# theteamatx/x-edr-trajectory-planning

Hardware: AMD Instinct MI355X
Metric: time-optimal path timings/s (7-DOF, 2000 s-samples), 1/2/4/8 MI355X + %HBM roofline (higher is better)
Workload: dtype f64

## Files before the change

x-edr-trajectory-planning_amd/csrc/tpamd_device.h:

```cpp
#pragma once

#include <hip/hip_runtime.h>
#include <float.h>
#include <stdint.h>

namespace tpamd {

constexpr double kTiny = 2.220446049250313e-16 * 1e5;
constexpr double kMaxSd2 = 1e6;

enum : uint8_t { kBndNone = 0, kBndSource = 1, kBndSink = 2, kBndTrajectory = 4 };
enum : uint8_t { kBndEqualsZ00 = 8, kBndTypeMask = 7 };

enum : uint32_t {
  kErrInfeasible = 1u,
  kErrSRange = 2u,
  kErrSdStartNeg = 4u,
  kErrLowerGeUpper = 8u,
  kErrTooFew = 16u,
  kErrSkip = 32u
};

__device__ __forceinline__ bool is_tiny(double v) { return fabs(v) < kTiny; }
__device__ __forceinline__ double qnan() { return __longlong_as_double(0x7ff8000000000000LL); }

__device__ __forceinline__ int status_from_bits(uint32_t bits) {
  if (bits & kErrInfeasible) return 2;
  if (bits & kErrSRange) return 3;
  if (bits & kErrSdStartNeg) return 4;
  if (bits & kErrLowerGeUpper) return 5;
  if (bits & kErrTooFew) return 6;
  return 0;
}


struct LdsRows {
  const double *A, *B, *LO, *HI;
  int stride;
  int lim_stride;
  __device__ __forceinline__ double a(int c) const { return A[c * stride]; }
  __device__ __forceinline__ double b(int c) const { return B[c * stride]; }
  __device__ __forceinline__ double lo(int c) const { return LO[c * lim_stride]; }
  __device__ __forceinline__ double hi(int c) const { return HI[c * lim_stride]; }
};

struct LdsRowsJoint {
  const double *Q1, *Q2;
  const double *lim_lo, *lim_hi;
  int stride, D;
  int E = 0;
  const double *X = nullptr;
  __device__ __forceinline__ double a(int c) const { return c < D ? Q1[c * stride] : 0.0; }
  __device__ __forceinline__ double b(int c) const {
    if (c < D) return Q2[c * stride];
    if (c >= 2 * D) return X[(c - 2 * D) * stride];
    const double v = Q1[(c - D) * stride];
    return v * v;
  }
  __device__ __forceinline__ double lo(int c) const { return lim_lo[c]; }
  __device__ __forceinline__ double hi(int c) const { return lim_hi[c]; }
};

struct JointRowsAt {
  const double *q12;
  const double *lim_lo, *lim_hi;
  int D;
  int E = 0;
  __device__ __forceinline__ double a(int c) const { return c < D ? q12[2 * c] : 0.0; }
  __device__ __forceinline__ double b(int c) const {
    if (c < D) return q12[2 * c + 1];
    if (c >= 2 * D) return q12[c];
    const double v = q12[2 * (c - D)];
    return v * v;
  }
  __device__ __forceinline__ double lo(int c) const { return lim_lo[c]; }
  __device__ __forceinline__ double hi(int c) const { return lim_hi[c]; }
};

struct GlobalRowsAt {
  const double *A, *B, *LO, *HI;
  __device__ __forceinline__ double a(int c) const { return A[c]; }
  __device__ __forceinline__ double b(int c) const { return B[c]; }
  __device__ __forceinline__ double lo(int c) const { return LO[c]; }
  __device__ __forceinline__ double hi(int c) const { return HI[c]; }
};

template <class R>
__device__ __forceinline__ bool rows_valid(const R &r, int C, double sdd, double sd2) {
  for (int i = 0; i < C; i++) {
    const double v = r.a(i) * sdd + r.b(i) * sd2;
// ... 79 lines not shown
    double bs[D], hi[D];
#pragma unroll
    for (int j = 0; j < D; j++) { bs[j] = b[j] * sd2; hi[j] = lim_hi[j]; }
#pragma unroll
    for (int i = 0; i < D; i++) {
      const double A = a[i];
      if (!is_tiny(A)) {
#pragma unroll
        for (int w = 0; w < 2; w++) {
          const double lim = w ? hi[i] : -hi[i];
          const double sddi = (lim - bs[i]) / A;
          if ((fabs(sddi) <= DBL_MAX) && ((sddi > smax) || (sddi < smin))) {
            bool bad = false;
#pragma unroll
            for (int j = 0; j < D; j++) {
              const double v = a[j] * sddi + bs[j];
              bad = bad | (fabs(v) - kTiny > hi[j]);
            }
            if (!bad) {
              if (sddi > smax) smax = sddi;
              if (sddi < smin) smin = sddi;
            }
          }
        }
      }
    }
  }
  if (smax == -DBL_MAX) smax = 0;
  if (smin == DBL_MAX) smin = 0;
  *sdd_max = smax;
  *sdd_min = smin;
}

template <int D>
__device__ __forceinline__ void find_sdd_both_joint_screened(const double (&a)[D], const double (&b)[D],
                                                             const double *Q1, const double *Q2, int stride,
                                                             const double *lim_hi, double sd2,
                                                             double *sdd_max, double *sdd_min) {
  double smax = -DBL_MAX, smin = DBL_MAX;
  bool vel_bad = false;
#pragma unroll
  for (int j = 0; j < D; j++) {
    const double v = (a[j] * a[j]) * sd2;
    vel_bad = vel_bad | (v + kTiny < 0.0) | (v - kTiny > lim_hi[D + j]);
  }
  const bool vel_ok = !vel_bad;
  if (vel_ok) {
    double bs[D], hi[D], c_lo[D], c_hi[D];
    double Lmax = -DBL_MAX, Umin = DBL_MAX;
#pragma unroll
    for (int j = 0; j < D; j++) {
      bs[j] = b[j] * sd2;
      hi[j] = lim_hi[j];
      const double r = __builtin_amdgcn_rcp(a[j]);
      c_lo[j] = (-hi[j] - bs[j]) * r;
      c_hi[j] = (hi[j] - bs[j]) * r;
      const bool counts = !is_tiny(a[j]);
      const double pad = kTiny * fabs(r);
      const double l = fmin(c_lo[j], c_hi[j]) - pad, u = fmax(c_lo[j], c_hi[j]) + pad;
      Lmax = (counts & (l > Lmax)) ? l : Lmax;
      Umin = (counts & (u < Umin)) ? u : Umin;
    }
    unsigned survivors = 0;
#pragma unroll
    for (int i = 0; i < D; i++) {
      const bool counts = !is_tiny(a[i]);
#pragma unroll
      for (int w = 0; w < 2; w++) {
        const double c = w ? c_hi[i] : c_lo[i];
        const double mg = 1e-6 * (fabs(Lmax) + fabs(Umin) + fabs(c)) + 1e-290;
        const bool out = (c < Lmax - mg) | (c > Umin + mg);
        survivors |= (counts & !out) ? (1u << (2 * i + w)) : 0u;
      }
    }
    while (__any(survivors != 0u)) {
      const bool live = survivors != 0u;
      const int slot = live ? (__ffs((int)survivors) - 1) : 0;
      survivors &= survivors - 1u;
      const int i = slot >> 1;
      const double A = Q1[i * stride];
      const double lim = (slot & 1) ? lim_hi[i] : -lim_hi[i];
      const double sddi = (lim - Q2[i * stride] * sd2) / A;
      if (live && (fabs(sddi) <= DBL_MAX) && ((sddi > smax) || (sddi < smin))) {
        bool bad = false;
#pragma unroll
        for (int j = 0; j < D; j++) {
          const double v = a[j] * sddi + bs[j];
          bad = bad | (fabs(v) - kTiny > hi[j]);
        }
        if (!bad) {
          if (sddi > smax) smax = sddi;
          if (sddi < smin) smin = sddi;
        }
      }
    }
  }
  if (smax == -DBL_MAX) smax = 0;
  if (smin == DBL_MAX) smin = 0;
  *sdd_max = smax;
  *sdd_min = smin;
}

template <int WORDS>
struct SlotSet {
  uint64_t w[WORDS];
  __device__ __forceinline__ void clear() {
#pragma unroll
    for (int i = 0; i < WORDS; i++) w[i] = 0;
  }
  __device__ __forceinline__ void fill(int n) {
#pragma unroll
    for (int i = 0; i < WORDS; i++) {
      const int lo = i * 64;
      w[i] = (n >= lo + 64) ? ~0ull : (n > lo ? ((1ull << (n - lo)) - 1ull) : 0ull);
    }
// ... 54 lines not shown
__device__ __forceinline__ bool lp_cannot_pass(double num, double den, double lo_lim,
                                               double hi_lim) {
  const double tmp_apx = num * __builtin_amdgcn_rcp(den);
  return (tmp_apx > hi_lim + fabs(hi_lim) * 1e-6) || (tmp_apx < lo_lim - fabs(lo_lim) * 1e-6);
}

template <class R>
__device__ __forceinline__ bool lp_pair_optimal(const R &r, int s1, int s2) {
  const int first = s1 >> 1, second = s2 >> 1;
  const bool first_upper = !(s1 & 1), second_upper = !(s2 & 1);
  const double a1 = r.a(first), a2 = r.a(second);
  const double denom = a2 * r.b(first) - a1 * r.b(second);
  const double t1 = denom * a1;
  const double t2 = denom * (-a2);
  const bool c1 = second_upper ? (t1 <= 0) : (t1 >= 0);
  const bool c2 = first_upper ? (t2 <= 0) : (t2 >= 0);
  return !(fabs(denom) < kTiny) & c1 & c2;
}

template <int WORDS, class R, int SD = 0, int SC = 0>
__device__ void lp_find_max_sd2(const R &r, int C, double *sd2max, double *sddmax,
                                double *sd2zero, int b_only_from = -1,
                                const double *ra = nullptr, const double *rb = nullptr) {
  typedef SlotSet<WORDS> Set;
  Set cset, act;
  cset.fill(2 * C);
  if (b_only_from >= 0) cset.drop_lower_from(b_only_from, C);
  act.clear();

  auto vel_b = [&](int c) -> double {
    if (SD > 0 && c < 2 * SD) { const double v = ra[c - SD]; return v * v; }
    return r.b(c);
  };
  double sd2 = DBL_MAX, sdd = 0.0;
  double hi_w = (sd2 + kTiny) + fabs(sd2 + kTiny) * 1e-6;
  auto step2_row = [&](int c, double Bc) {
    const bool pos = Bc > kTiny, neg = Bc < -kTiny;
    const double lim = pos ? r.hi(c) : r.lo(c);
    const double ap = lim * __builtin_amdgcn_rcp(Bc);
    if ((pos | neg) & !((ap > hi_w) | (ap < 0.0))) {
      const double invB = 1.0 / Bc;
      const double tmp = lim * invB;
      if (tmp < (sd2 + kTiny) && tmp > 0) {
        if (tmp < sd2 - kTiny) act.clear();
        act.set(2 * c + (pos ? 0 : 1));
        sd2 = tmp;
        hi_w = (sd2 + kTiny) + fabs(sd2 + kTiny) * 1e-6;
      }
    }
  };
  if (SD > 0) {
#pragma unroll
    for (int c = 0; c < SC; c++) step2_row(c, (c < SD) ? rb[c < SD ? c : 0] : vel_b(c));
  } else {
    for (int c = 0; c < C; c++) step2_row(c, r.b(c));
  }
  if (sd2 > kMaxSd2 || !act.any()) {
    *sd2zero = kMaxSd2;
    *sd2max = kMaxSd2;
    *sddmax = 0.0;
    return;
  }
  *sd2zero = sd2;

  int search = act.next(0);
  if (act.count() >= 2) {
    double best_slope = fabs(r.a(search >> 1) * (1.0 / r.b(search >> 1)));
    for (int s1 = act.next(0); s1 >= 0; s1 = act.next(s1 + 1)) {
      const double slope = fabs(r.a(s1 >> 1) * (1.0 / r.b(s1 >> 1)));
      if (slope < best_slope) {
        best_slope = slope;
        search = s1;
      }
      for (int s2 = act.next(s1 + 1); s2 >= 0; s2 = act.next(s2 + 1)) {
        if (lp_pair_optimal(r, s1, s2)) {
          *sd2max = sd2;
          *sddmax = 0.0;
          return;
        }
      }
    }
  }
  cset.remove(act);

  for (int loop = 0; loop < C; loop++) {
    if (search < 0) break;
    const int sc = search >> 1;
    const double As = r.a(sc);
    if (fabs(As) < kTiny) {
      *sd2max = sd2;
      *sddmax = sdd;
      return;
    }
    const double invA = 1.0 / As;
    const double b = -r.b(sc) * invA;
    const double a = (search & 1) ? r.lo(sc) * invA : r.hi(sc) * invA;

    act.clear();
    double next_sd2 = DBL_MAX, next_sdd = 0.0;
    const double lo_w = sd2 - fabs(sd2) * 1e-6;
    double up_w = (next_sd2 + kTiny) + fabs(next_sd2 + kTiny) * 1e-6;
    auto visit = [&](int s, bool member, double Ac, double Brow, double lim) {
      const double Bc = Ac * b + Brow;
      const double num = lim - Ac * a;
      const double tmp_apx = num * __builtin_amdgcn_rcp(Bc);
      if (!(member & !(fabs(Bc) < kTiny) & !((tmp_apx > up_w) | (tmp_apx < lo_w)))) return;
      const double invB = 1.0 / Bc;
      const double tmp = num * invB;
      if (tmp < (next_sd2 + kTiny) && tmp > sd2) {
        if (tmp < next_sd2 - kTiny) act.clear();
        act.set(s);
        next_sd2 = tmp;
        next_sdd = a + b * next_sd2;
        up_w = (next_sd2 + kTiny) + fabs(next_sd2 + kTiny) * 1e-6;
      }
    };
    if (SD > 0) {
#pragma unroll
      for (int c = 0; c < SC; c++) {
        const double Ac = (c < SD) ? ra[c < SD ? c : 0] : r.a(c);
        const double Brow = (c < SD) ? rb[c < SD ? c : 0] : vel_b(c);
        visit(2 * c, cset.has(2 * c), Ac, Brow, r.hi(c));
        if (!(b_only_from >= 0 && c >= b_only_from)) visit(2 * c + 1, cset.has(2 * c + 1), Ac, Brow, r.lo(c));
      }
    } else {
      for (int s = cset.next(0); s >= 0; s = cset.next(s + 1)) {
        const int c = s >> 1;
        visit(s, true, r.a(c), r.b(c), (s & 1) ? r.lo(c) : r.hi(c));
      }
    }
    if (!act.any()) {
      *sd2max = *sd2zero;
      *sddmax = 0.0;
      return;
    }
    const int old_search = search;
    search = -1;
    double best_slope = DBL_MAX;
    for (int s1 = act.next(0); s1 >= 0; s1 = act.next(s1 + 1)) {
      const int c1 = s1 >> 1;
      const double Ac = r.a(c1);
      const double slope = fabs(Ac * (1.0 / (Ac * b + r.b(c1))));
      if (slope < best_slope) {
        best_slope = slope;
        search = s1;
      }
      bool opt = false;
      for (int s2 = act.next(s1 + 1); s2 >= 0 && !opt; s2 = act.next(s2 + 1))
        opt = lp_pair_optimal(r, s1, s2);
      if (!opt) opt = lp_pair_optimal(r, s1, old_search);
      if (opt) {
        *sd2max = next_sd2;
        *sddmax = next_sdd;
        if (next_sd2 > kMaxSd2) {
          *sd2max = kMaxSd2;
          *sddmax = 0.0;
// ... 122 lines not shown
```

x-edr-trajectory-planning_amd/csrc/tpamd_capi.hip:

```cpp
#include "../../include/tpamd.h"

#include <hip/hip_runtime.h>

#include <algorithm>
#include <cmath>
#include <cstdio>
#include <cstdlib>
#include <cstring>
#include <mutex>
#include <new>
#include <vector>

#include "tpamd_kernels.h"
#include "tpamd_launch.h"
#include "tpamd_planner_set.h"
#include "tpamd_readout.h"
#include "tpamd_rescale.h"
#include "tpamd_buffer.h"
#include "tpamd_stop.h"
#include "tpamd_switch.h"
#include "tpamd_fit.h"
#include "tpamd_pose_fit.h"
#include "tpamd_sweep_joint.h"

// ... 326 lines not shown
};

struct DeviceScope {
  int prev = -1;
  hipError_t err;
  explicit DeviceScope(int device) {
    if (hipGetDevice(&prev) != hipSuccess) prev = -1;
    err = (prev == device) ? hipSuccess : hipSetDevice(device);
    if (prev == device) prev = -1;
  }
  ~DeviceScope() {
    if (prev >= 0) (void)hipSetDevice(prev);
  }
};
#define TPAMD_ON_DEVICE(e)          \
  DeviceScope device_scope_((e)->device); \
  HIPCHK(device_scope_.err)

constexpr int kMaxDevices = 64;
std::mutex g_config_mutex;
bool g_device_configured[kMaxDevices] = {};

template <typename K>
hipError_t allow_big_lds(K kernel, int bytes = 160 * 1024) {
  return hipFuncSetAttribute(reinterpret_cast<const void *>(kernel),
                             hipFuncAttributeMaxDynamicSharedMemorySize, bytes);
}

int configure_kernels_for_device(int device) {
  if (device < 0 || device >= kMaxDevices) return TPAMD_E_INVALID_ARGUMENT;
  std::lock_guard<std::mutex> lock(g_config_mutex);
  if (g_device_configured[device]) return 0;
#define TPAMD_BIG_LDS(...) HIPCHK(allow_big_lds(__VA_ARGS__))
  TPAMD_BIG_LDS(k_sample_lp_joint<1, 0>);
  TPAMD_BIG_LDS(k_sample_lp_joint<1, 3>);
  TPAMD_BIG_LDS(k_sample_lp_joint<1, 4>);
  TPAMD_BIG_LDS(k_sample_lp_joint<1, 5>);
  TPAMD_BIG_LDS(k_sample_lp_joint<1, 6>);
  TPAMD_BIG_LDS(k_sample_lp_joint<1, 7>);
  TPAMD_BIG_LDS(k_sample_lp_joint<1, 8>);
  TPAMD_BIG_LDS(k_sample_lp_joint<1, 14>);
  TPAMD_BIG_LDS(k_sample_lp_joint_wide<1, 14>);
  TPAMD_BIG_LDS(k_lp_rows<1>);
  TPAMD_BIG_LDS(k_lp_rows<2>);
  TPAMD_BIG_LDS(k_sweep<JointSource>);
  TPAMD_BIG_LDS(k_sweep<GenericSource>);
#define TPAMD_CONFIGURE_SWEEP(D, E) HIPCHK((configure_sweep_joint<D, E>()));
  TPAMD_SWEEP_INSTANCES(TPAMD_CONFIGURE_SWEEP)
#undef TPAMD_CONFIGURE_SWEEP
  TPAMD_BIG_LDS(k_cartesian_lp<1, 6>);
  TPAMD_BIG_LDS(k_cartesian_lp<1, 7>);
  TPAMD_BIG_LDS(k_resample_skip, 128 * 1024);
#undef TPAMD_BIG_LDS
  g_device_configured[device] = true;
  return 0;
}

bool has_joint_sweep(int D) { return (D >= 3 && D <= 8) || D == 14; }

template <class Source>
bool launch_sweep(hipStream_t st, int B, int N, int max_loops, const Source &src,
                  const Workspace &ws, const tpamd_path_outputs *out, bool ) {
  const size_t lds = (2 * (size_t)N + 64) * sizeof(double);
  hipLaunchKernelGGL((k_sweep<Source>), dim3(B), dim3(64), lds, st, N, max_loops, src, ws,
                     out->time, out->s, out->sd, out->sdd, out->last_extremal_index,
                     out->max_time_increment, out->status);
  return false;
}

template <>
bool launch_sweep<JointSource>(hipStream_t st, int B, int N, int max_loops, const JointSource &src,
                               const Workspace &ws, const tpamd_path_outputs *out,
                               bool force_generic) {
#define TPAMD_LAUNCH_JOINT(DD)                                              \
  do {                                                                      \
// ... 213 lines not shown
  return rc;
}

size_t tpamd_engine_workspace_bytes(const tpamd_engine *e) { return e ? e->ws_buf.bytes : 0; }

}

namespace {
int joint_args(const tpamd_joint_batch *bt, const tpamd_joint_inputs *in, const tpamd_path_outputs *out) {
  const int D = bt->num_dofs, N = bt->num_samples, P = bt->num_points;
  if (D < 1 || D > 16 || N < 3 || N > 8192 || P < 3) return TPAMD_E_UNSUPPORTED;
  if (!in->knots || !in->control_points || !in->max_velocity || !in->max_acceleration ||
      !in->path_start || !in->delta || !in->sd_start || !in->time_start || !out->time ||
      !out->s || !out->sd || !out->sdd || !out->status)
    return TPAMD_E_INVALID_ARGUMENT;
  return 0;
}

int solve_joint(tpamd_engine *e, const tpamd_joint_batch *bt, const tpamd_joint_inputs *in,
                const tpamd_path_outputs *out, void *hip_stream, const PlanParams *plan,
                bool allow_pipelining = true) {
  if (!e || !bt || !in || !out) return TPAMD_E_INVALID_ARGUMENT;
  const int B = bt->num_paths, D = bt->num_dofs, N = bt->num_samples, P = bt->num_points;
  if (B <= 0) return B == 0 ? 0 : TPAMD_E_INVALID_ARGUMENT;
  if (int rc = joint_args(bt, in, out)) return rc;
  TPAMD_ON_DEVICE(e);
  hipStream_t st = (hipStream_t)hip_stream;
  const int C = 2 * D;
  bool piped = e->pipelining != 0 && plan == nullptr && allow_pipelining;
  if (piped && stream_is_capturing(st)) piped = false;
  int tpb = piped ? 128 : (D <= 7 ? 256 : (D < 14 ? 128 : 64));
  if (!piped && in->num_samples_per_path && tpb > e->k1_tpb_ragged) tpb = e->k1_tpb_ragged;
  if (e->k1_tpb == 64 || e->k1_tpb == 128 || e->k1_tpb == 256) tpb = e->k1_tpb;
  const size_t lds = ((size_t)(P + 3) + (size_t)P * D + 2 * C + 2 * (size_t)D * tpb) * 8;
  if (lds > 160 * 1024) return TPAMD_E_UNSUPPORTED;
  if (piped) select_slot(e, 1 - e->slot);
  const int slot = e->slot;
  SlotGuard slot_guard(e, st, true, !piped);
  int rc = ensure_workspace(e, B, N, C);
  if (rc) return rc;
  e->last_B = B; e->last_N = N; e->last_time = out->time;
  e->ws.ns = in->num_samples_per_path;
  e->ws.amax = in->max_acceleration;
  e->ws.np = plan ? plan->np : nullptr;
  e->ws.p_stride = (plan && plan->np) ? plan->K - 3 : P;
  int32_t *order = const_cast<int32_t *>(e->ws.order);
  const bool ordered = in->num_samples_per_path != nullptr && B > 1 && e->order_ragged && plan == nullptr;
  if (!ordered) e->ws.order = nullptr;
  const Workspace &ws = e->ws;
  const int max_loops = bt->max_solver_loops > 0 ? bt->max_solver_loops : 0;
  hipStream_t fs = st;
  if (piped) {
    fs = e->aux;
    HIPCHK(hipStreamWaitEvent(fs, e->ev_sweep[slot], 0));
  }
  const bool do_front = e->phase != 2, do_back = e->phase != 1;
  if (do_front && piped && e->front_delay_us > 0)
    hipLaunchKernelGGL(k_delay, dim3(1), dim3(64), 0, fs, e->front_delay_us * 100);
  if (do_front) {
    Timer t(e, fs, KI_SETUP);
    hipLaunchKernelGGL(k_setup_joint, dim3((B + 127) / 128), dim3(128), 0, fs, B, N, D,
                       bt->constraint_safety, in->max_velocity, in->max_acceleration,
                       in->path_start, in->delta, in->sd_start, in->sdd_start, in->time_start,
                       ws);
    if (plan)
      hipLaunchKernelGGL(k_plan_mark_skipped, dim3((B + 127) / 128), dim3(128), 0, fs, *plan, ws);
    if (ordered)
      hipLaunchKernelGGL(k_order_paths, dim3(1), dim3(1024), 0, fs, B, N, in->num_samples_per_path, order);
  }
  if (do_front && e->front_wait) HIPCHK(hipStreamWaitEvent(fs, e->front_wait, 0));
  if (do_front) {
    Timer t(e, fs, KI_SAMPLE_LP);
    const dim3 grid((N + tpb - 1) / tpb, B);
#define TPAMD_K1(DD)                                                                         \
  hipLaunchKernelGGL((k_sample_lp_joint<1, DD>), grid, dim3(tpb), lds, fs, N, D, P, in->knots, \
                     in->control_points, out->q, ws)
    if (D == 7 && !e->force_generic) TPAMD_K1(7);
    else if (D == 6 && !e->force_generic) TPAMD_K1(6);
    else if (D == 14 && !e->force_generic)
      hipLaunchKernelGGL((k_sample_lp_joint_wide<1, 14>), grid, dim3(tpb), lds, fs, N, D, P, in->knots,
                         in->control_points, out->q, ws);
    else if (D == 3 && !e->force_generic) TPAMD_K1(3);
    else if (D == 4 && !e->force_generic) TPAMD_K1(4);
    else if (D == 5 && !e->force_generic) TPAMD_K1(5);
    else if (D == 8 && !e->force_generic) TPAMD_K1(8);
    else TPAMD_K1(0);
#undef TPAMD_K1
    if (plan) hipLaunchKernelGGL(k_plan_project, dim3((B + 127) / 128), dim3(128), 0, fs, *plan, ws);
  }
  if (do_front && e->front_record) HIPCHK(hipEventRecord(e->front_record, fs));
  if (!do_back) {
    HIPCHK(hipGetLastError());
    return 0;
  }
  for (hipEvent_t ev : e->back_wait) HIPCHK(hipStreamWaitEvent(st, ev, 0));
  const bool deferred = piped && e->pipelining == 2;
  hipStream_t caller = st;
  if (piped) {
    HIPCHK(hipEventRecord(e->ev_front[slot], fs));
    if (deferred) {
      HIPCHK(hipEventRecord(e->ev_call[slot], caller));
      st = e->sweep_stream[slot];
      HIPCHK(hipStreamWaitEvent(st, e->ev_call[slot], 0));
    }
    HIPCHK(hipStreamWaitEvent(st, e->ev_front[slot], 0));
  }
  JointSource src;
  src.q12 = ws.q12; src.lim = ws.lim; src.D = D;
  bool fused = false;
  rc = run_boundary_and_sweep(e, st, B, N, max_loops, src, out, &fused);
  if (rc) {
    if (piped) (void)hipEventRecord(e->ev_sweep[slot], st);
    return rc;
  }
  if (!fused && (out->qd || out->qdd)) {
    Timer t(e, st, KI_EPILOGUE);
    const size_t total = (size_t)B * N * D;
    hipLaunchKernelGGL(k_epilogue, dim3((unsigned)((total + 255) / 256)), dim3(256), 0, st, B, N,
                       D, ws.q12, out->sd, out->sdd, in->max_acceleration, out->status, ws.ns,
// ... 1114 lines not shown
  int rc = s.upload(e->stage, st);
  if (rc) return rc;
  rc = tpamd_fastest_stop_device(e, &da, st);
  return rc ? rc : s.download(st);
}

int tpamd_debug_copy_boundary(tpamd_engine *e, int B, int N, double *sd2_max, double *sdd_max,
                              double *sdd_min, double *sd2_zero, uint8_t *type, double *sd2) {
  if (!e || B != e->last_B || N != e->last_N) return TPAMD_E_INVALID_ARGUMENT;
  TPAMD_ON_DEVICE(e);
  HIPCHK(hipDeviceSynchronize());
  const size_t n = (size_t)B * N;
  if (sd2_max) HIPCHK(hipMemcpy(sd2_max, e->ws.m, n * 8, hipMemcpyDeviceToHost));
  if (sdd_max) HIPCHK(hipMemcpy(sdd_max, e->ws.X, n * 8, hipMemcpyDeviceToHost));
  if (sdd_min) HIPCHK(hipMemcpy(sdd_min, e->ws.Y, n * 8, hipMemcpyDeviceToHost));
  if (sd2_zero) HIPCHK(hipMemcpy(sd2_zero, e->ws.z0, n * 8, hipMemcpyDeviceToHost));
  if (type) {
    HIPCHK(hipMemcpy(type, e->ws.type, n, hipMemcpyDeviceToHost));
    for (size_t i = 0; i < n; i++) type[i] &= kBndTypeMask;
  }
  if (sd2) HIPCHK(hipMemcpy(sd2, e->ws.sd2, n * 8, hipMemcpyDeviceToHost));
  return 0;
}

void tpamd_debug_keep_boundary(tpamd_engine *e, int on) {
  if (e) e->keep_boundary = on != 0;
}

int tpamd_debug_kernel_vgprs(tpamd_engine *e, int which) {
  if (!e || which < 0 || which > 1) return TPAMD_E_INVALID_ARGUMENT;
  TPAMD_ON_DEVICE(e);
  hipFuncAttributes attr;
  if (which == 0)
    HIPCHK(hipFuncGetAttributes(&attr, reinterpret_cast<const void *>(&k_sample_lp_joint<1, 7>)));
  else
    HIPCHK((sweep_joint_attributes<7, 0>(&attr)));
  return attr.numRegs;
}

int tpamd_debug_copy_diag(tpamd_engine *e, int B, long long *out) {
  if (!e || !out || B != e->last_B) return TPAMD_E_INVALID_ARGUMENT;
  TPAMD_ON_DEVICE(e);
  HIPCHK(hipDeviceSynchronize());
#ifdef TPAMD_K1_STUDY
  HIPCHK(hipMemcpy(out, e->ws.diag, (size_t)B * 64 * 8, hipMemcpyDeviceToHost));
#else
  HIPCHK(hipMemcpy2D(out, 64 * 8, e->ws.diag, kDiagRow * 8, 64 * 8, (size_t)B, hipMemcpyDeviceToHost));
#endif
  return 0;
}

int tpamd_debug_copy_diag_ext(tpamd_engine *e, int B, long long *out) {
  if (!e || !out || B != e->last_B) return TPAMD_E_INVALID_ARGUMENT;
  TPAMD_ON_DEVICE(e);
  HIPCHK(hipDeviceSynchronize());
  HIPCHK(hipMemcpy2D(out, 2 * kDiagExt * 8, e->ws.diag + 64, kDiagRow * 8, 2 * kDiagExt * 8, (size_t)B,
                     hipMemcpyDeviceToHost));
  return 0;
}

void tpamd_profile_enable(tpamd_engine *e, int enable) {
  if (e) e->profile = (enable == 2) ? 2 : (enable != 0 ? 1 : 0);
}

void tpamd_profile_reset(tpamd_engine *e) {
  if (!e) return;
  DeviceScope scope(e->device);
// ... 1866 lines not shown
```

x-edr-trajectory-planning_amd/csrc/tpamd_kernels.h:

```cpp
#pragma once

#include "tpamd_device.h"
#include "tpamd_cartesian_window.h"
#include "tpamd_quat.h"

namespace tpamd {

constexpr int kDiagExt = 16;
constexpr int kDiagRow = 64 + 2 * kDiagExt;

struct Workspace {
  double *ds, *s_start, *s_end, *sd_start, *sdd_start, *t_start, *delta;
  uint32_t *err_bits;
  const int32_t *ns;
  const double *amax;
  const int32_t *order;
  double *lim;
  double *q12;
  double *m0, *z0, *X0, *Y0, *Xz, *Yz;
  uint8_t *at0;
  uint8_t *fix_flag;
  double *fix_val;
  double *m, *X, *Y;
  uint8_t *type;
// ... 144 lines not shown

static __global__ void k_setup_rows(int B, int N, const double *s_start, const double *s_end,
                             const double *sd_start, const double *sdd_start,
                             const double *t_start, Workspace ws) {
  const int b = blockIdx.x * blockDim.x + threadIdx.x;
  if (b >= B) return;
  uint32_t bits = 0;
  if (s_start[b] >= s_end[b]) bits |= kErrSRange;
  if (sd_start[b] < 0) bits |= kErrSdStartNeg;
  if (N < 2) bits |= kErrTooFew;
  ws.err_bits[b] = bits;
  ws.s_start[b] = s_start[b];
  ws.s_end[b] = s_end[b];
  ws.ds[b] = (s_end[b] - s_start[b]) / (N - 1);
  ws.sd_start[b] = sd_start[b];
  ws.sdd_start[b] = sdd_start ? sdd_start[b] : 0.0;
  ws.t_start[b] = t_start[b];
}

template <int WORDS, bool JOINT, class R>
__device__ __forceinline__ void boundary_point(const R &r, int C, size_t o, Workspace ws) {
  double sd2max, sddmax, sd2zero;
  lp_find_max_sd2<WORDS>(r, C, &sd2max, &sddmax, &sd2zero);
  double x0, y0;
  if (JOINT) find_sdd_both_joint(r, C / 2, sd2max, &x0, &y0);
  else find_sdd_both(r, C, sd2max, &x0, &y0);
  ws.m0[o] = sd2max;
  ws.z0[o] = sd2zero;
  ws.X0[o] = x0;
  ws.Y0[o] = y0;
  ws.at0[o] = fabs(sd2max - sd2zero) < kTiny;
}

template <int WORDS, int DT>
__device__ __forceinline__ void sample_lp_joint_body(int N, int D_rt, int P, const double *knots_g,
                                                     const double *cps_g, double *q_out,
                                                     const Workspace &ws) {
  extern __shared__ double lds[];
#ifdef TPAMD_K1_PRIO
  __builtin_amdgcn_s_setprio(TPAMD_K1_PRIO);
#endif
#ifdef TPAMD_K1_STUDY
  if (threadIdx.x == 0) {
    unsigned long long t;
    asm volatile("s_memrealtime %0\n\ts_waitcnt lgkmcnt(0)" : "=s"(t)::"memory");
    unsigned xcc;
    asm volatile("s_getreg_b32 %0, hwreg(HW_REG_XCC_ID)" : "=s"(xcc));
    reinterpret_cast<unsigned long long *>(ws.diag)[2 * (blockIdx.y * gridDim.x + blockIdx.x)] = t | ((unsigned long long)(xcc & 15u) << 60);
  }
#endif
  const int TPB = blockDim.x;
  const int tid = threadIdx.x;
  const int b = blockIdx.y;
  const int K = P + 3;
  const int D = DT ? DT : D_rt;
  const int C = 2 * D;
  if ((int)(blockIdx.x * TPB) >= path_samples(ws, b, N)) return;
  const int Ps = ws.np ? ws.p_stride : P;
  const int Pb = ws.np ? ws.np[b] : P;
  const int Kb = Pb + 3;
  double q1r[DT ? DT : 1], q2r[DT ? DT : 1];
  double *s_knots = lds;
  double *s_cp = s_knots + K;
  double *s_lo = s_cp + P * D;
  double *s_hi = s_lo + C;
  double *s_Q1 = s_hi + C;
  double *s_Q2 = s_Q1 + (size_t)D * TPB;
  for (int k = tid; k < Kb; k += TPB) s_knots[k] = knots_g[(size_t)b * (Ps + 3) + k];
  for (int k = tid; k < Pb * D; k += TPB) s_cp[k] = cps_g[(size_t)b * Ps * D + k];
  for (int k = tid; k < 2 * C; k += TPB) s_lo[k] = ws.lim[(size_t)b * 2 * C + k];
  __syncthreads();
  const int i0 = blockIdx.x * TPB;
  const int i = i0 + tid;
  const int Nb = path_samples(ws, b, N);
  const bool live = i < Nb;
  const size_t o = (size_t)b * N + i;

  const double path_start = ws.s_start[b];
  const double delta = ws.delta[b];
  const double k0 = s_knots[0], kend = s_knots[Kb - 1];
  const double parameter = path_start + i * delta;
  double *Q1 = s_Q1 + tid, *Q2 = s_Q2 + tid;
  if (!live) {
  } else if (parameter < kend + delta) {
    double u = parameter;
    if (u < k0) u = k0;
    if (kend < u) u = kend;
    const int span = knot_span_deg2(s_knots, Kb, u);
    double ders[3][3];
    basis_ders_deg2(s_knots, span, u, ders);
    const double *p0 = s_cp + (size_t)(span - 2) * D, *p1 = p0 + D, *p2 = p1 + D;
#pragma unroll
    for (int d = 0; d < D; d++) {
      double v0 = 0.0, v1 = 0.0, v2 = 0.0;
      v0 += ders[0][0] * p0[d]; v0 += ders[0][1] * p1[d]; v0 += ders[0][2] * p2[d];
      v1 += ders[1][0] * p0[d]; v1 += ders[1][1] * p1[d]; v1 += ders[1][2] * p2[d];
      v2 += ders[2][0] * p0[d]; v2 += ders[2][1] * p1[d]; v2 += ders[2][2] * p2[d];
      if (q_out) q_out[o * D + d] = v0;
      Q1[d * TPB] = v1;
      Q2[d * TPB] = v2;
      if (DT) { q1r[d] = v1; q2r[d] = v2; }
    }
  } else {
    const double *pl = s_cp + (size_t)(Pb - 1) * D;
#pragma unroll
    for (int d = 0; d < D; d++) {
      if (q_out) q_out[o * D + d] = pl[d];
      Q1[d * TPB] = 0.0;
      Q2[d * TPB] = 0.0;
      if (DT) { q1r[d] = 0.0; q2r[d] = 0.0; }
    }
  }
  __syncthreads();
  {
    const int nvalid = min(TPB, Nb - i0);
    double2 *recs = reinterpret_cast<double2 *>(ws.q12 + ((size_t)b * N + i0) * (C + 2));
    const int pairs = D + 1;
    for (int c = tid; c < nvalid * pairs; c += TPB) {
      const int sm = c / pairs, pr = c - sm * pairs;
      recs[c] = (pr < D) ? make_double2(s_Q1[pr * TPB + sm], s_Q2[pr * TPB + sm]) : make_double2(0.0, 0.0);
    }
  }
  if (!live) return;
  LdsRowsJoint r;
  r.Q1 = Q1; r.Q2 = Q2; r.lim_lo = s_lo; r.lim_hi = s_hi; r.stride = TPB; r.D = D;
  if (DT) {
    double sd2max, sddmax, sd2zero, x0, y0;
    lp_find_max_sd2<WORDS, LdsRowsJoint, DT, 2 * DT>(r, C, &sd2max, &sddmax, &sd2zero, D,
                                                     q1r, q2r);
    find_sdd_both_joint_screened<(DT ? DT : 1)>(q1r, q2r, Q1, Q2, TPB, s_hi, sd2max, &x0, &y0);
    ws.m0[o] = sd2max;
    ws.z0[o] = sd2zero;
    ws.X0[o] = x0;
    ws.Y0[o] = y0;
    ws.at0[o] = fabs(sd2max - sd2zero) < kTiny;
  } else {
    boundary_point<WORDS, true>(r, C, o, ws);
  }
#ifdef TPAMD_K1_STUDY
  __syncthreads();
  if (threadIdx.x == 0) {
    unsigned long long t;
    asm volatile("s_memrealtime %0\n\ts_waitcnt lgkmcnt(0)" : "=s"(t)::"memory");
    reinterpret_cast<unsigned long long *>(ws.diag)[2 * (blockIdx.y * gridDim.x + blockIdx.x) + 1] = t;
  }
#endif
}

#ifdef TPAMD_K1_STUDY
#define TPAMD_K1_STUDY_REGS __attribute__((amdgpu_waves_per_eu(5, 5)))
#else
#define TPAMD_K1_STUDY_REGS
#endif
template <int WORDS, int DT>
__global__ void TPAMD_K1_STUDY_REGS k_sample_lp_joint(int N, int D_rt, int P, const double *knots_g,
                                  const double *cps_g, double *q_out, Workspace ws) {
  sample_lp_joint_body<WORDS, DT>(N, D_rt, P, knots_g, cps_g, q_out, ws);
}
template <int WORDS, int DT>
__global__ void __launch_bounds__(256) __attribute__((amdgpu_waves_per_eu(1, 2)))
k_sample_lp_joint_wide(int N, int D_rt, int P, const double *knots_g, const double *cps_g,
                       double *q_out, Workspace ws) {
  sample_lp_joint_body<WORDS, DT>(N, D_rt, P, knots_g, cps_g, q_out, ws);
}

static __global__ void k_sample_only(int N, int D, int P, const double *knots_g, const double *cps_g,
                              const double *path_start, const double *delta_g, double *q,
                              double *q1, double *q2) {
  extern __shared__ double lds[];
  const int TPB = blockDim.x, tid = threadIdx.x, b = blockIdx.y, K = P + 3;
  double *s_knots = lds, *s_cp = lds + K;
  for (int k = tid; k < K; k += TPB) s_knots[k] = knots_g[(size_t)b * K + k];
  for (int k = tid; k < P * D; k += TPB) s_cp[k] = cps_g[(size_t)b * P * D + k];
  __syncthreads();
  const int i = blockIdx.x * TPB + tid;
  if (i >= N) return;
  const size_t o = ((size_t)b * N + i) * D;
  const double delta = delta_g[b];
  const double k0 = s_knots[0], kend = s_knots[K - 1];
  const double parameter = path_start[b] + i * delta;
  if (parameter < kend + delta) {
    double u = parameter;
    if (u < k0) u = k0;
    if (kend < u) u = kend;
    const int span = knot_span_deg2(s_knots, K, u);
    double ders[3][3];
    basis_ders_deg2(s_knots, span, u, ders);
    const double *p0 = s_cp + (size_t)(span - 2) * D, *p1 = p0 + D, *p2 = p1 + D;
    for (int d = 0; d < D; d++) {
      double v0 = 0.0, v1 = 0.0, v2 = 0.0;
      v0 += ders[0][0] * p0[d]; v0 += ders[0][1] * p1[d]; v0 += ders[0][2] * p2[d];
      v1 += ders[1][0] * p0[d]; v1 += ders[1][1] * p1[d]; v1 += ders[1][2] * p2[d];
      v2 += ders[2][0] * p0[d]; v2 += ders[2][1] * p1[d]; v2 += ders[2][2] * p2[d];
      q[o + d] = v0; q1[o + d] = v1; q2[o + d] = v2;
    }
  } else {
// ... 174 lines not shown
#pragma unroll
  for (int r = 0; r < 6; r++) v6[r] = s_Q2[r * TPB + tid];
  __syncthreads();
#pragma unroll
  for (int d = 0; d < D; d++) Q2[d * TPB] = q2r[d];
  const double bt = (v6[0] * v6[0] + v6[1] * v6[1]) + v6[2] * v6[2];
  const double br = (v6[3] * v6[3] + v6[4] * v6[4]) + v6[5] * v6[5];
  X[0] = bt;
  X[TPB] = br;
  __syncthreads();
  {
    const int nvalid = min(TPB, N - i0);
    double2 *recs = reinterpret_cast<double2 *>(ws.q12 + ((size_t)b * N + i0) * (C + 2));
    constexpr int pairs = D + 2;
    for (int c = tid; c < nvalid * pairs; c += TPB) {
      const int sm = c / pairs, pr = c - sm * pairs;
      double2 v = make_double2(0.0, 0.0);
      if (pr < D) v = make_double2(s_Q1[pr * TPB + sm], s_Q2[pr * TPB + sm]);
      else if (pr == D) v = make_double2(s_X[sm], s_X[TPB + sm]);
      recs[c] = v;
    }
  }
  if (!live) return;
  LdsRowsJoint r;
  r.Q1 = Q1; r.Q2 = Q2; r.lim_lo = s_lo; r.lim_hi = s_hi; r.stride = TPB; r.D = D;
  r.E = 2; r.X = X;
  double sd2max, sddmax, sd2zero, x0 = 0.0, y0 = 0.0;
  lp_find_max_sd2<WORDS, LdsRowsJoint, D, 2 * D + 2>(r, C, &sd2max, &sddmax, &sd2zero, D,
                                                     q1r, q2r);
  {
    const double vt = bt * sd2max, vr = br * sd2max;
    const bool ok = !(vt + kTiny < s_lo[2 * D] || vt - kTiny > s_hi[2 * D]) &&
                    !(vr + kTiny < s_lo[2 * D + 1] || vr - kTiny > s_hi[2 * D + 1]);
    if (ok) find_sdd_both_joint_screened<D>(q1r, q2r, Q1, Q2, TPB, s_hi, sd2max, &x0, &y0);
  }
  ws.m0[o] = sd2max;
  ws.z0[o] = sd2zero;
  ws.X0[o] = x0;
  ws.Y0[o] = y0;
  ws.at0[o] = fabs(sd2max - sd2zero) < kTiny;
}

template <int WORDS>
__global__ void k_lp_rows(int N, int C, const double *Ag, const double *Bg, const double *LOg,
                          const double *HIg, Workspace ws) {
  extern __shared__ double lds[];
  const int TPB = blockDim.x;
  const int tid = threadIdx.x;
  const int b = blockIdx.y;
  double *s_A = lds, *s_B = s_A + (size_t)C * TPB, *s_LO = s_B + (size_t)C * TPB,
         *s_HI = s_LO + (size_t)C * TPB;
  const int i0 = blockIdx.x * TPB;
  const int nvalid = min(TPB, path_samples(ws, b, N) - i0);
  const size_t base = ((size_t)b * N + i0) * C;
  for (int k = tid; k < nvalid * C; k += TPB) {
    const int s = k / C, c = k - s * C;
    s_A[c * TPB + s] = Ag[base + k];
    s_B[c * TPB + s] = Bg[base + k];
    s_LO[c * TPB + s] = LOg[base + k];
    s_HI[c * TPB + s] = HIg[base + k];
  }
  __syncthreads();
  if (tid >= nvalid) return;
  const size_t o = (size_t)b * N + i0 + tid;
  LdsRows r;
  r.A = s_A + tid; r.B = s_B + tid; r.LO = s_LO + tid; r.HI = s_HI + tid;
  r.stride = TPB; r.lim_stride = TPB;
// ... 1112 lines not shown
```

Measured before the change: 2.125 million.

## Add fast path for isolated velocity-cap constraint in LP max-sd2 search

In the LP solver, velocity-cap rows (those at or after b_only_from) get a cheap pre-scan using approximate reciprocals. The scan finds the tightest cap and checks whether it is clearly separated from the next one. When it is isolated, that single constraint is applied directly in both the step-2 scan and the visit loop, and the full per-row exact divisions are skipped. A cold fallback path, with an asm barrier to keep it out of the hot code, handles the non-isolated case. This adds branching and register pressure, and relies on the tolerance margin to keep results matching the full scan.

New measurement: 2.149 million (median of 6 runs). +1.2%, better.

```diff
diff --git a/x-edr-trajectory-planning_amd/csrc/tpamd_device.h b/x-edr-trajectory-planning_amd/csrc/tpamd_device.h
--- a/x-edr-trajectory-planning_amd/csrc/tpamd_device.h
+++ b/x-edr-trajectory-planning_amd/csrc/tpamd_device.h
@@ -370,6 +370,14 @@
     if (SD > 0 && c < 2 * SD) { const double v = ra[c - SD]; return v * v; }
     return r.b(c);
   };
+  auto vel_b_cold = [&](int c) -> double {
+    if (SD > 0 && c < 2 * SD) {
+      double v = ra[c - SD];
+      asm volatile("" : "+v"(v));
+      return v * v;
+    }
+    return r.b(c);
+  };
   double sd2 = DBL_MAX, sdd = 0.0;
   double hi_w = (sd2 + kTiny) + fabs(sd2 + kTiny) * 1e-6;
   auto step2_row = [&](int c, double Bc) {
@@ -387,9 +395,52 @@
       }
     }
   };
+  constexpr bool kVelCap = SD > 0;
+  double vc_T = 0.0;
+  bool vc_isolated = false;
+  int vc_slot = 0;
   if (SD > 0) {
-#pragma unroll
-    for (int c = 0; c < SC; c++) step2_row(c, (c < SD) ? rb[c < SD ? c : 0] : vel_b(c));
+    const int vel_from = (kVelCap && b_only_from >= 0) ? b_only_from : SC;
+#pragma unroll
+    for (int c = 0; c < SC; c++)
+      if (c < vel_from) step2_row(c, (c < SD) ? rb[c < SD ? c : 0] : vel_b(c));
+    if (vel_from < SC) {
+      double e1 = DBL_MAX, e2 = DBL_MAX;
+      int slot = -1;
+#pragma unroll
+      for (int c = 0; c < SC; c++) {
+        if (c < vel_from) continue;
+        const double Bc = vel_b(c);
+        const bool pos = Bc > kTiny;
+        const double ap = r.hi(c) * __builtin_amdgcn_rcp(Bc);
+        const bool first = pos & (ap < e1);
+        const double other = first ? e1 : ((pos & (ap == ap)) ? ap : -DBL_MAX);
+        if (!(fabs(Bc) < kTiny) & (other < e2)) e2 = other;
+        if (first) { e1 = ap; slot = 2 * c; }
+      }
+      double Bm = 1.0, him = 0.0;
+#pragma unroll
+      for (int c = 0; c < SC; c++) {
+        if (c < vel_from) continue;
+        const bool is = slot == 2 * c;
+        Bm = is ? vel_b(c) : Bm;
+        him = is ? r.hi(c) : him;
+      }
+      vc_T = him * (1.0 / Bm);
+      vc_isolated = (slot >= 0) & (e2 * (1.0 - 2e-6) > e1 * (1.0 + 2e-6) + 2.0 * kTiny);
+      vc_slot = slot < 0 ? 0 : slot;
+      const bool one = vc_isolated & (vc_T > 0.0);
+      if (one & (vc_T < (sd2 + kTiny))) {
+        if (vc_T < sd2 - kTiny) act.clear();
+        act.set(vc_slot);
+        sd2 = vc_T;
+      }
+      if (!one) {
+#pragma unroll
+        for (int c = 0; c < SC; c++)
+          if (c >= vel_from) step2_row(c, vel_b_cold(c));
+      }
+    }
   } else {
     for (int c = 0; c < C; c++) step2_row(c, r.b(c));
   }
@@ -454,12 +505,30 @@
       }
     };
     if (SD > 0) {
-#pragma unroll
-      for (int c = 0; c < SC; c++) {
+      const int vel_from = (kVelCap && b_only_from >= 0) ? b_only_from : SC;
+      auto visit_row = [&](int c) {
         const double Ac = (c < SD) ? ra[c < SD ? c : 0] : r.a(c);
-        const double Brow = (c < SD) ? rb[c < SD ? c : 0] : vel_b(c);
+        const double Brow = (c < SD) ? rb[c < SD ? c : 0] : (c >= vel_from ? vel_b_cold(c) : vel_b(c));
         visit(2 * c, cset.has(2 * c), Ac, Brow, r.hi(c));
         if (!(b_only_from >= 0 && c >= b_only_from)) visit(2 * c + 1, cset.has(2 * c + 1), Ac, Brow, r.lo(c));
+      };
+#pragma unroll
+      for (int c = 0; c < SC; c++)
+        if (c < vel_from) visit_row(c);
+      if (vel_from < SC) {
+        const bool one = vc_isolated & (fabs(a) <= DBL_MAX) & (fabs(b) <= DBL_MAX) & cset.has(vc_slot) &
+                         (vc_T > sd2);
+        if (one & (vc_T < (next_sd2 + kTiny))) {
+          if (vc_T < next_sd2 - kTiny) act.clear();
+          act.set(vc_slot);
+          next_sd2 = vc_T;
+          next_sdd = a + b * next_sd2;
+        }
+        if (!one) {
+#pragma unroll
+          for (int c = 0; c < SC; c++)
+            if (c >= vel_from) visit_row(c);
+        }
       }
     } else {
       for (int s = cset.next(0); s >= 0; s = cset.next(s + 1)) {
```

## Store per-sample q1/q2 as interleaved double2 image in LDS with compile-time TPB

Applied to the files above, without the earlier changes.

Replaces the SoA Q1/Q2 LDS arrays in the joint sample+LP kernel with an interleaved double2 per-thread image, padded so D+1 pairs form an aligned record (for D=7, groups of 8 threads plus a zero pair). The q12 record write-out then becomes a straight, coalesced copy instead of a strided gather with div/mod. The block size becomes a template parameter, so loops unroll and 3x kernel instantiations are built. This risks LDS bank conflicts from the stride-D accesses in the LP solve, and the larger binary adds compile cost.

Measured after the change: 2.160 million before, 2.179 million after, median of 6. Within noise of the previous version (+0.9%).

```diff
diff --git a/x-edr-trajectory-planning_amd/csrc/tpamd_capi.hip b/x-edr-trajectory-planning_amd/csrc/tpamd_capi.hip
--- a/x-edr-trajectory-planning_amd/csrc/tpamd_capi.hip
+++ b/x-edr-trajectory-planning_amd/csrc/tpamd_capi.hip
@@ -382,15 +382,21 @@
   std::lock_guard<std::mutex> lock(g_config_mutex);
   if (g_device_configured[device]) return 0;
 #define TPAMD_BIG_LDS(...) HIPCHK(allow_big_lds(__VA_ARGS__))
-  TPAMD_BIG_LDS(k_sample_lp_joint<1, 0>);
-  TPAMD_BIG_LDS(k_sample_lp_joint<1, 3>);
-  TPAMD_BIG_LDS(k_sample_lp_joint<1, 4>);
-  TPAMD_BIG_LDS(k_sample_lp_joint<1, 5>);
-  TPAMD_BIG_LDS(k_sample_lp_joint<1, 6>);
-  TPAMD_BIG_LDS(k_sample_lp_joint<1, 7>);
-  TPAMD_BIG_LDS(k_sample_lp_joint<1, 8>);
-  TPAMD_BIG_LDS(k_sample_lp_joint<1, 14>);
-  TPAMD_BIG_LDS(k_sample_lp_joint_wide<1, 14>);
+#define TPAMD_K1_BIG_LDS(DD)                      \
+  TPAMD_BIG_LDS(k_sample_lp_joint<1, DD, 64>);    \
+  TPAMD_BIG_LDS(k_sample_lp_joint<1, DD, 128>);   \
+  TPAMD_BIG_LDS(k_sample_lp_joint<1, DD, 256>)
+  TPAMD_K1_BIG_LDS(0);
+  TPAMD_K1_BIG_LDS(3);
+  TPAMD_K1_BIG_LDS(4);
+  TPAMD_K1_BIG_LDS(5);
+  TPAMD_K1_BIG_LDS(6);
+  TPAMD_K1_BIG_LDS(7);
+  TPAMD_K1_BIG_LDS(8);
+#undef TPAMD_K1_BIG_LDS
+  TPAMD_BIG_LDS(k_sample_lp_joint_wide<1, 14, 64>);
+  TPAMD_BIG_LDS(k_sample_lp_joint_wide<1, 14, 128>);
+  TPAMD_BIG_LDS(k_sample_lp_joint_wide<1, 14, 256>);
   TPAMD_BIG_LDS(k_lp_rows<1>);
   TPAMD_BIG_LDS(k_lp_rows<2>);
   TPAMD_BIG_LDS(k_sweep<JointSource>);
@@ -670,7 +676,10 @@
   int tpb = piped ? 128 : (D <= 7 ? 256 : (D < 14 ? 128 : 64));
   if (!piped && in->num_samples_per_path && tpb > e->k1_tpb_ragged) tpb = e->k1_tpb_ragged;
   if (e->k1_tpb == 64 || e->k1_tpb == 128 || e->k1_tpb == 256) tpb = e->k1_tpb;
-  const size_t lds = ((size_t)(P + 3) + (size_t)P * D + 2 * C + 2 * (size_t)D * tpb) * 8;
+  const int k1_dt = (!e->force_generic && ((D >= 3 && D <= 8) || D == 14)) ? D : 0;
+  const size_t k1_image_pairs = k1_dt == 3 ? K1Image<3>::pairs(D, tpb) : k1_dt == 7 ? K1Image<7>::pairs(D, tpb)
+                                                                                     : K1Image<0>::pairs(D, tpb);
+  const size_t lds = ((size_t)(P + 3) + (size_t)P * D + 2 * C) * 8 + k1_image_pairs * 16;
   if (lds > 160 * 1024) return TPAMD_E_UNSUPPORTED;
   if (piped) select_slot(e, 1 - e->slot);
   const int slot = e->slot;
@@ -710,19 +719,26 @@
   if (do_front) {
     Timer t(e, fs, KI_SAMPLE_LP);
     const dim3 grid((N + tpb - 1) / tpb, B);
-#define TPAMD_K1(DD)                                                                         \
-  hipLaunchKernelGGL((k_sample_lp_joint<1, DD>), grid, dim3(tpb), lds, fs, N, D, P, in->knots, \
+#define TPAMD_K1_LAUNCH(KERNEL, DD, TT)                                                       \
+  hipLaunchKernelGGL((KERNEL<1, DD, TT>), grid, dim3(TT), lds, fs, N, D, P, in->knots,         \
                      in->control_points, out->q, ws)
-    if (D == 7 && !e->force_generic) TPAMD_K1(7);
-    else if (D == 6 && !e->force_generic) TPAMD_K1(6);
-    else if (D == 14 && !e->force_generic)
-      hipLaunchKernelGGL((k_sample_lp_joint_wide<1, 14>), grid, dim3(tpb), lds, fs, N, D, P, in->knots,
-                         in->control_points, out->q, ws);
-    else if (D == 3 && !e->force_generic) TPAMD_K1(3);
-    else if (D == 4 && !e->force_generic) TPAMD_K1(4);
-    else if (D == 5 && !e->force_generic) TPAMD_K1(5);
-    else if (D == 8 && !e->force_generic) TPAMD_K1(8);
+#define TPAMD_K1_OF(KERNEL, DD)                                \
+  do {                                                         \
+    if (tpb == 64) TPAMD_K1_LAUNCH(KERNEL, DD, 64);            \
+    else if (tpb == 128) TPAMD_K1_LAUNCH(KERNEL, DD, 128);     \
+    else TPAMD_K1_LAUNCH(KERNEL, DD, 256);                     \
+  } while (0)
+#define TPAMD_K1(DD) TPAMD_K1_OF(k_sample_lp_joint, DD)
+    if (k1_dt == 7) TPAMD_K1(7);
+    else if (k1_dt == 6) TPAMD_K1(6);
+    else if (k1_dt == 14) TPAMD_K1_OF(k_sample_lp_joint_wide, 14);
+    else if (k1_dt == 3) TPAMD_K1(3);
+    else if (k1_dt == 4) TPAMD_K1(4);
+    else if (k1_dt == 5) TPAMD_K1(5);
+    else if (k1_dt == 8) TPAMD_K1(8);
     else TPAMD_K1(0);
+#undef TPAMD_K1_OF
+#undef TPAMD_K1_LAUNCH
 #undef TPAMD_K1
     if (plan) hipLaunchKernelGGL(k_plan_project, dim3((B + 127) / 128), dim3(128), 0, fs, *plan, ws);
   }
@@ -1903,7 +1919,7 @@
   TPAMD_ON_DEVICE(e);
   hipFuncAttributes attr;
   if (which == 0)
-    HIPCHK(hipFuncGetAttributes(&attr, reinterpret_cast<const void *>(&k_sample_lp_joint<1, 7>)));
+    HIPCHK(hipFuncGetAttributes(&attr, reinterpret_cast<const void *>(&k_sample_lp_joint<1, 7, 128>)));
   else
     HIPCHK((sweep_joint_attributes<7, 0>(&attr)));
   return attr.numRegs;
diff --git a/x-edr-trajectory-planning_amd/csrc/tpamd_device.h b/x-edr-trajectory-planning_amd/csrc/tpamd_device.h
--- a/x-edr-trajectory-planning_amd/csrc/tpamd_device.h
+++ b/x-edr-trajectory-planning_amd/csrc/tpamd_device.h
@@ -56,6 +56,26 @@
     if (c >= 2 * D) return X[(c - 2 * D) * stride];
     const double v = Q1[(c - D) * stride];
     return v * v;
+  }
+  __device__ __forceinline__ double lo(int c) const { return lim_lo[c]; }
+  __device__ __forceinline__ double hi(int c) const { return lim_hi[c]; }
+  __device__ __forceinline__ double2 pair(int i) const { return make_double2(Q1[i * stride], Q2[i * stride]); }
+};
+
+struct LdsPairsJoint {
+  const double2 *P;
+  const double *lim_lo, *lim_hi;
+  int D;
+  __device__ __forceinline__ double2 pair(int i) const { return P[i]; }
+  __device__ __forceinline__ double a(int c) const {
+    const bool acc = c < D;
+    const double2 p = P[acc ? c : c - D];
+    return acc ? p.x : 0.0;
+  }
+  __device__ __forceinline__ double b(int c) const {
+    const bool acc = c < D;
+    const double2 p = P[acc ? c : c - D];
+    return acc ? p.y : p.x * p.x;
   }
   __device__ __forceinline__ double lo(int c) const { return lim_lo[c]; }
   __device__ __forceinline__ double hi(int c) const { return lim_hi[c]; }
@@ -201,9 +221,9 @@
   *sdd_min = smin;
 }
 
-template <int D>
+template <int D, class R>
 __device__ __forceinline__ void find_sdd_both_joint_screened(const double (&a)[D], const double (&b)[D],
-                                                             const double *Q1, const double *Q2, int stride,
+                                                             const R &rows,
                                                              const double *lim_hi, double sd2,
                                                              double *sdd_max, double *sdd_min) {
   double smax = -DBL_MAX, smin = DBL_MAX;
@@ -247,9 +267,10 @@
       const int slot = live ? (__ffs((int)survivors) - 1) : 0;
       survivors &= survivors - 1u;
       const int i = slot >> 1;
-      const double A = Q1[i * stride];
+      const double2 qi = rows.pair(i);
+      const double A = qi.x;
       const double lim = (slot & 1) ? lim_hi[i] : -lim_hi[i];
-      const double sddi = (lim - Q2[i * stride] * sd2) / A;
+      const double sddi = (lim - qi.y * sd2) / A;
       if (live && (fabs(sddi) <= DBL_MAX) && ((sddi > smax) || (sddi < smin))) {
         bool bad = false;
 #pragma unroll
diff --git a/x-edr-trajectory-planning_amd/csrc/tpamd_kernels.h b/x-edr-trajectory-planning_amd/csrc/tpamd_kernels.h
--- a/x-edr-trajectory-planning_amd/csrc/tpamd_kernels.h
+++ b/x-edr-trajectory-planning_amd/csrc/tpamd_kernels.h
@@ -200,11 +200,26 @@
   ws.at0[o] = fabs(sd2max - sd2zero) < kTiny;
 }
 
-template <int WORDS, int DT>
+template <int DT>
+struct K1Image {
+  static constexpr int S = DT + 1;
+  static constexpr bool kZero = DT > 0 && (S & (S - 1)) == 0 && S <= 64;
+  static constexpr int kGroup = kZero ? 64 / S : 1;
+  static constexpr int kGroupPairs = kZero ? kGroup * DT + 1 : DT;
+  __host__ __device__ static constexpr int pairs(int D, int tpb) {
+    return kZero ? (tpb / kGroup) * kGroupPairs : tpb * (D | 1);
+  }
+  __device__ __forceinline__ static int home(int t, int D) {
+    return kZero ? (t / kGroup) * kGroupPairs + (t % kGroup) * DT : t * (D | 1);
+  }
+};
+
+template <int WORDS, int DT, int TPB>
 __device__ __forceinline__ void sample_lp_joint_body(int N, int D_rt, int P, const double *knots_g,
                                                      const double *cps_g, double *q_out,
                                                      const Workspace &ws) {
-  extern __shared__ double lds[];
+  extern __shared__ double2 lds_k1[];
+  typedef K1Image<DT> Image;
 #ifdef TPAMD_K1_PRIO
   __builtin_amdgcn_s_setprio(TPAMD_K1_PRIO);
 #endif
@@ -217,7 +232,6 @@
     reinterpret_cast<unsigned long long *>(ws.diag)[2 * (blockIdx.y * gridDim.x + blockIdx.x)] = t | ((unsigned long long)(xcc & 15u) << 60);
   }
 #endif
-  const int TPB = blockDim.x;
   const int tid = threadIdx.x;
   const int b = blockIdx.y;
   const int K = P + 3;
@@ -228,12 +242,11 @@
   const int Pb = ws.np ? ws.np[b] : P;
   const int Kb = Pb + 3;
   double q1r[DT ? DT : 1], q2r[DT ? DT : 1];
-  double *s_knots = lds;
+  double2 *s_img = lds_k1;
+  double *s_knots = reinterpret_cast<double *>(s_img + Image::pairs(D, TPB));
   double *s_cp = s_knots + K;
   double *s_lo = s_cp + P * D;
   double *s_hi = s_lo + C;
-  double *s_Q1 = s_hi + C;
-  double *s_Q2 = s_Q1 + (size_t)D * TPB;
   for (int k = tid; k < Kb; k += TPB) s_knots[k] = knots_g[(size_t)b * (Ps + 3) + k];
   for (int k = tid; k < Pb * D; k += TPB) s_cp[k] = cps_g[(size_t)b * Ps * D + k];
   for (int k = tid; k < 2 * C; k += TPB) s_lo[k] = ws.lim[(size_t)b * 2 * C + k];
@@ -248,7 +261,11 @@
   const double delta = ws.delta[b];
   const double k0 = s_knots[0], kend = s_knots[Kb - 1];
   const double parameter = path_start + i * delta;
-  double *Q1 = s_Q1 + tid, *Q2 = s_Q2 + tid;
+  double2 *Q = s_img + Image::home(tid, D);
+  if (Image::kZero)
+    s_img[(tid / Image::kGroup) * Image::kGroupPairs + Image::kGroup * DT] = make_double2(0.0, 0.0);
+  else if (D % 2 == 0)
+    Q[D] = make_double2(0.0, 0.0);
   if (!live) {
   } else if (parameter < kend + delta) {
     double u = parameter;
@@ -265,8 +282,7 @@
       v1 += ders[1][0] * p0[d]; v1 += ders[1][1] * p1[d]; v1 += ders[1][2] * p2[d];
       v2 += ders[2][0] * p0[d]; v2 += ders[2][1] * p1[d]; v2 += ders[2][2] * p2[d];
       if (q_out) q_out[o * D + d] = v0;
-      Q1[d * TPB] = v1;
-      Q2[d * TPB] = v2;
+      Q[d] = make_double2(v1, v2);
       if (DT) { q1r[d] = v1; q2r[d] = v2; }
     }
   } else {
@@ -274,8 +290,7 @@
 #pragma unroll
     for (int d = 0; d < D; d++) {
       if (q_out) q_out[o * D + d] = pl[d];
-      Q1[d * TPB] = 0.0;
-      Q2[d * TPB] = 0.0;
+      Q[d] = make_double2(0.0, 0.0);
       if (DT) { q1r[d] = 0.0; q2r[d] = 0.0; }
     }
   }
@@ -284,19 +299,49 @@
     const int nvalid = min(TPB, Nb - i0);
     double2 *recs = reinterpret_cast<double2 *>(ws.q12 + ((size_t)b * N + i0) * (C + 2));
     const int pairs = D + 1;
-    for (int c = tid; c < nvalid * pairs; c += TPB) {
-      const int sm = c / pairs, pr = c - sm * pairs;
-      recs[c] = (pr < D) ? make_double2(s_Q1[pr * TPB + sm], s_Q2[pr * TPB + sm]) : make_double2(0.0, 0.0);
+    const int lim = nvalid * pairs;
+    if constexpr (Image::kZero) {
+      constexpr int S = Image::S;
+      const int pr = tid % S;
+      const int within = pr < DT ? ((tid / S) % Image::kGroup) * DT + pr : Image::kGroup * DT;
+      const double2 *src = s_img + (tid / 64) * Image::kGroupPairs + within;
+      constexpr int step = (TPB / 64) * Image::kGroupPairs;
+      if (nvalid == TPB) {
+#pragma unroll
+        for (int k = 0; k < S; k++) recs[tid + k * TPB] = src[k * step];
+      } else {
+#pragma unroll
+        for (int k = 0; k < S; k++)
+          if (tid + k * TPB < lim) recs[tid + k * TPB] = src[k * step];
+      }
+    } else if constexpr (DT > 0 && DT % 2 == 0) {
+#pragma unroll
+      for (int k = 0; k < DT + 1; k++)
+        if (tid + k * TPB < lim) recs[tid + k * TPB] = s_img[tid + k * TPB];
+    } else if constexpr (DT > 0) {
+#pragma unroll
+      for (int k = 0; k < DT + 1; k++) {
+        const int c = tid + k * TPB;
+        const int sm = c / (DT + 1), pr = c - sm * (DT + 1);
+        if (c < lim) recs[c] = (pr < DT) ? s_img[sm * DT + pr] : make_double2(0.0, 0.0);
+      }
+    } else if (D % 2 == 0) {
+      for (int c = tid; c < lim; c += TPB) recs[c] = s_img[c];
+    } else {
+      for (int c = tid; c < lim; c += TPB) {
+        const int sm = c / pairs, pr = c - sm * pairs;
+        recs[c] = (pr < D) ? s_img[sm * D + pr] : make_double2(0.0, 0.0);
+      }
     }
   }
   if (!live) return;
-  LdsRowsJoint r;
-  r.Q1 = Q1; r.Q2 = Q2; r.lim_lo = s_lo; r.lim_hi = s_hi; r.stride = TPB; r.D = D;
+  LdsPairsJoint r;
+  r.P = Q; r.lim_lo = s_lo; r.lim_hi = s_hi; r.D = D;
   if (DT) {
     double sd2max, sddmax, sd2zero, x0, y0;
-    lp_find_max_sd2<WORDS, LdsRowsJoint, DT, 2 * DT>(r, C, &sd2max, &sddmax, &sd2zero, D,
-                                                     q1r, q2r);
-    find_sdd_both_joint_screened<(DT ? DT : 1)>(q1r, q2r, Q1, Q2, TPB, s_hi, sd2max, &x0, &y0);
+    lp_find_max_sd2<WORDS, LdsPairsJoint, DT, 2 * DT>(r, C, &sd2max, &sddmax, &sd2zero, D,
+                                                      q1r, q2r);
+    find_sdd_both_joint_screened<(DT ? DT : 1)>(q1r, q2r, r, s_hi, sd2max, &x0, &y0);
     ws.m0[o] = sd2max;
     ws.z0[o] = sd2zero;
     ws.X0[o] = x0;
@@ -320,16 +365,16 @@
 #else
 #define TPAMD_K1_STUDY_REGS
 #endif
-template <int WORDS, int DT>
+template <int WORDS, int DT, int TPB>
 __global__ void TPAMD_K1_STUDY_REGS k_sample_lp_joint(int N, int D_rt, int P, const double *knots_g,
                                   const double *cps_g, double *q_out, Workspace ws) {
-  sample_lp_joint_body<WORDS, DT>(N, D_rt, P, knots_g, cps_g, q_out, ws);
-}
-template <int WORDS, int DT>
+  sample_lp_joint_body<WORDS, DT, TPB>(N, D_rt, P, knots_g, cps_g, q_out, ws);
+}
+template <int WORDS, int DT, int TPB>
 __global__ void __launch_bounds__(256) __attribute__((amdgpu_waves_per_eu(1, 2)))
 k_sample_lp_joint_wide(int N, int D_rt, int P, const double *knots_g, const double *cps_g,
                        double *q_out, Workspace ws) {
-  sample_lp_joint_body<WORDS, DT>(N, D_rt, P, knots_g, cps_g, q_out, ws);
+  sample_lp_joint_body<WORDS, DT, TPB>(N, D_rt, P, knots_g, cps_g, q_out, ws);
 }
 
 static __global__ void k_sample_only(int N, int D, int P, const double *knots_g, const double *cps_g,
@@ -570,7 +615,7 @@
     const double vt = bt * sd2max, vr = br * sd2max;
     const bool ok = !(vt + kTiny < s_lo[2 * D] || vt - kTiny > s_hi[2 * D]) &&
                     !(vr + kTiny < s_lo[2 * D + 1] || vr - kTiny > s_hi[2 * D + 1]);
-    if (ok) find_sdd_both_joint_screened<D>(q1r, q2r, Q1, Q2, TPB, s_hi, sd2max, &x0, &y0);
+    if (ok) find_sdd_both_joint_screened<D>(q1r, q2r, r, s_hi, sd2max, &x0, &y0);
   }
   ws.m0[o] = sd2max;
   ws.z0[o] = sd2zero;
```
